# yycho0108/qpwcnet

Hardware: AMD Instinct MI355X
Metric: image-pairs/sec at 256x512 fp32 (higher is better)
Workload: dtype f32; 1 GPU; BASELINE configs[1]: full 6-level PWC-Net (qpwcnet build_flower) inference, batch 8 per GPU, 256x512 fp32, channels_last, d=4 cost volume + WarpV2; global_batch=8, batch_per_gpu=8, parallelism=dp1 (pairs sharded, RCCL all-gather of the 6 per-level EPE), hipgraph=True

## Files before the change

include/qpwc.h:

```cpp
#ifndef QPWC_H_
#define QPWC_H_

#include <stddef.h>
#include <stdint.h>

#ifdef __cplusplus
extern "C" {
#endif

#define QPWC_VERSION 200

#define QPWC_NHWC 0
#define QPWC_NCHW 1

#define QPWC_F32 0
#define QPWC_F16 1

#define QPWC_WARP_CLAMP 0
#define QPWC_WARP_TFWARP 1

#define QPWC_BCAST_B 1
#define QPWC_BCAST_H 2
#define QPWC_BCAST_W 4

// ... 138 lines not shown
int qpwc_invert_flow_fwd(const void* flow, void* out, int B, int H, int W, int layout, int dtype,
                         void* stream);

int qpwc_occlusion_fwd(const void* flow, void* out, int B, int H, int W, int layout, int dtype,
                       void* stream);

int qpwc_conv3x3_mish_fwd(const void* x, const void* weight, const void* bias, void* out, int B, int H,
                          int W, int C, int pad_h, int pad_w, void* stream);

int qpwc_conv3x3_mish_x3_fwd(const void* x, const void* weight3, const void* bias, void* out, int B, int H,
                             int W, int C, int pad_h, int pad_w, void* stream);

int qpwc_split_bf16x3_fwd(const void* src, void* out, long long n, void* stream);

int qpwc_conv3x3_mish_f16_fwd(const void* x, const void* weight, const void* bias, void* out, int B, int H,
                              int W, int C, int pad_h, int pad_w, void* stream);

int qpwc_first_conv_mish_fwd(const void* pairs, const void* weight, const void* bias, void* out, int B,
                             int H, int W, int layout, void* stream);

int qpwc_first_conv_mish_f16_fwd(const void* pairs, const void* weight, const void* bias, void* out, int B,
                                 int H, int W, int layout, void* stream);

int qpwc_conv3x3s2_mish_fwd(const void* x_padded, const void* weight, const void* bias, void* out, int B,
                            int H, int W, void* stream);

int qpwc_conv3x3s2_mish_c_fwd(const void* x_padded, const void* weight, const void* bias, void* out, int B,
                              int H, int W, int C_in, void* stream);

int qpwc_conv3x3s2_mish_x3_fwd(const void* x_padded, const void* weight3, const void* bias, void* out, int B,
                               int H, int W, int C_in, void* stream);

int qpwc_conv3x3s2_mish_f16_fwd(const void* x_padded, const void* weight, const void* bias, void* out, int B,
                                int H, int W, int C_in, void* stream);

int qpwc_upconv4x4s2_mish_fwd(const void* x, const void* weight, const void* bias, void* out, int B, int H, int W,
                              int C, int F, int64_t out_pixel_stride, void* stream);

int qpwc_upconv4x4s2_mish_x3_fwd(const void* x, const void* weight3, const void* bias, void* out, int B, int H, int W,
                                 int C, int F, int64_t out_pixel_stride, void* stream);

int qpwc_upconv4x4s2_mish_f16_fwd(const void* x, const void* weight, const void* bias, void* out, int B, int H, int W,
                                  int C, int F, int64_t out_pixel_stride, void* stream);

int qpwc_upconv4x4s2_mish_cat_fwd(const void* x, const void* weight, const void* bias, const void* skip,
                                  int64_t skip_batch_stride, int64_t skip_row_stride, int64_t skip_pixel_stride, void* out,
// ... 11 lines not shown
```

qpwcnet_amd/_hip.py:

```python
import ctypes
import os

_HERE = os.path.dirname(os.path.abspath(__file__))
LIB_PATH = os.environ.get("QPWC_HIP_LIB") or os.path.join(_HERE, "csrc", "libqpwc_hip.so")

NHWC, NCHW = 0, 1
F32, F16 = 0, 1
WARP_CLAMP, WARP_TFWARP = 0, 1
BCAST_B, BCAST_H, BCAST_W = 1, 2, 4
LOSS_FLOW_MSE_V2, LOSS_FLOW_MSE, LOSS_FLOW_FINETUNE, LOSS_AUTORESIZE_MSE = 0, 1, 2, 3

E_NULL, E_LAYOUT, E_DTYPE, E_SHAPE, E_RANGE, E_MODE, E_ALIAS, E_LAUNCH, E_ALIGN, E_STRIDE, \
    E_NODEVICE = range(-1, -12, -1)
_ARGUMENT_ERRORS = {E_NULL, E_LAYOUT, E_DTYPE, E_SHAPE, E_RANGE, E_MODE, E_ALIAS, E_ALIGN, E_STRIDE}

SYMBOLS = (
    "qpwc_version", "qpwc_last_error", "qpwc_strerror", "qpwc_build_info", "qpwc_device_copy", "qpwc_clock_probe", "qpwc_layout_transpose_fwd", "qpwc_copy_pixels_fwd",
    "qpwc_cost_volume_fwd", "qpwc_cost_volume_fwd_strided", "qpwc_warp_fwd",
    "qpwc_warp_cost_volume_fwd", "qpwc_cost_volume_kernel", "qpwc_epe_workspace_floats", "qpwc_epe_fwd",
    "qpwc_dwconv3x3_fwd", "qpwc_flow_head_param_floats", "qpwc_flow_head_fwd", "qpwc_flow_head_up_fwd", "qpwc_pointwise_bias_fwd", "qpwc_optflow_tail_fwd", "qpwc_bias_mish_fwd",
    "qpwc_upsample2x_flow_fwd", "qpwc_epe_multi_workspace_floats", "qpwc_epe_multi_fwd", "qpwc_epe_multi_mixed_fwd",
    "qpwc_cost_volume_to_flow_fwd", "qpwc_sepconv3x3_fwd", "qpwc_sepconv3x3_f16_fwd", "qpwc_bias_mish_pad_fwd", "qpwc_split_frames_pad_fwd",
    "qpwc_invert_flow_fwd", "qpwc_occlusion_fwd", "qpwc_conv3x3_mish_fwd", "qpwc_conv3x3_mish_f16_fwd", "qpwc_conv3x3_mish_x3_fwd", "qpwc_split_bf16x3_fwd", "qpwc_sepconv3x3_x3_fwd", "qpwc_conv3x3s2_mish_x3_fwd", "qpwc_upconv4x4s2_mish_x3_fwd",
    "qpwc_first_conv_mish_fwd", "qpwc_first_conv_mish_f16_fwd", "qpwc_conv3x3s2_mish_fwd", "qpwc_conv3x3s2_mish_c_fwd", "qpwc_conv3x3s2_mish_f16_fwd", "qpwc_upconv4x4s2_mish_fwd", "qpwc_upconv4x4s2_mish_f16_fwd", "qpwc_upconv4x4s2_mish_cat_fwd", "qpwc_upconv4x4s2_mish_cat_f16_fwd",
    "qpwc_cost_volume_bwd", "qpwc_warp_bwd_workspace_floats", "qpwc_warp_bwd",
    "qpwc_loss_workspace_floats", "qpwc_loss_fwd", "qpwc_loss_fwd_kernel", "qpwc_loss_bwd",
)

_lib = None


def build(verbose=False):
    import subprocess
    cmd = ["make", "-C", os.path.join(_HERE, "csrc"), "-j4"]
    if not verbose:
        cmd.append("-s")
    subprocess.check_call(cmd)
    return LIB_PATH


def lib():
    global _lib
    if _lib is not None:
        return _lib
    if not os.path.exists(LIB_PATH):
        raise RuntimeError(
            "qpwcnet_amd: {} is missing -- build it with `make -C qpwcnet_amd/csrc` or "
# ... 69 lines not shown
    L.qpwc_cost_volume_to_flow_fwd.argtypes = [vp, vp, ci, ci, ci, ci, i64, ci, ci, vp]
    L.qpwc_cost_volume_to_flow_fwd.restype = ci
    L.qpwc_sepconv3x3_f16_fwd.restype = ci
    L.qpwc_bias_mish_pad_fwd.argtypes = [vp, vp, vp, ci, ci, ci, ci, ci, ci, i64, ci, vp]
    L.qpwc_bias_mish_pad_fwd.restype = ci
    L.qpwc_split_frames_pad_fwd.argtypes = [vp, vp, ci, ci, ci, ci, ci, ci, vp]
    L.qpwc_split_frames_pad_fwd.restype = ci
    L.qpwc_invert_flow_fwd.argtypes = [vp, vp, ci, ci, ci, ci, ci, vp]
    L.qpwc_invert_flow_fwd.restype = ci
    L.qpwc_occlusion_fwd.argtypes = [vp, vp, ci, ci, ci, ci, ci, vp]
    L.qpwc_occlusion_fwd.restype = ci
    L.qpwc_conv3x3_mish_f16_fwd.argtypes = [vp, vp, vp, vp, ci, ci, ci, ci, ci, ci, vp]
    L.qpwc_conv3x3_mish_f16_fwd.restype = ci
    L.qpwc_conv3x3_mish_fwd.argtypes = [vp, vp, vp, vp, ci, ci, ci, ci, ci, ci, vp]
    L.qpwc_conv3x3_mish_fwd.restype = ci
    L.qpwc_conv3x3_mish_x3_fwd.argtypes = [vp, vp, vp, vp, ci, ci, ci, ci, ci, ci, vp]
    L.qpwc_conv3x3_mish_x3_fwd.restype = ci
    L.qpwc_split_bf16x3_fwd.argtypes = [vp, vp, i64, vp]
    L.qpwc_split_bf16x3_fwd.restype = ci
    L.qpwc_first_conv_mish_fwd.argtypes = [vp, vp, vp, vp, ci, ci, ci, ci, vp]
    L.qpwc_first_conv_mish_fwd.restype = ci
    L.qpwc_first_conv_mish_f16_fwd.argtypes = L.qpwc_first_conv_mish_fwd.argtypes
    L.qpwc_first_conv_mish_f16_fwd.restype = ci
    L.qpwc_conv3x3s2_mish_fwd.argtypes = [vp, vp, vp, vp, ci, ci, ci, vp]
    L.qpwc_conv3x3s2_mish_fwd.restype = ci
    L.qpwc_conv3x3s2_mish_c_fwd.argtypes = [vp, vp, vp, vp, ci, ci, ci, ci, vp]
    L.qpwc_conv3x3s2_mish_c_fwd.restype = ci
    L.qpwc_conv3x3s2_mish_f16_fwd.argtypes = L.qpwc_conv3x3s2_mish_c_fwd.argtypes
    L.qpwc_conv3x3s2_mish_x3_fwd.argtypes = L.qpwc_conv3x3s2_mish_c_fwd.argtypes
    L.qpwc_conv3x3s2_mish_x3_fwd.restype = ci
    L.qpwc_conv3x3s2_mish_f16_fwd.restype = ci
    L.qpwc_upconv4x4s2_mish_fwd.argtypes = [vp, vp, vp, vp, ci, ci, ci, ci, ci, i64, vp]
    L.qpwc_upconv4x4s2_mish_fwd.restype = ci
    L.qpwc_upconv4x4s2_mish_f16_fwd.argtypes = L.qpwc_upconv4x4s2_mish_fwd.argtypes
    L.qpwc_upconv4x4s2_mish_x3_fwd.argtypes = L.qpwc_upconv4x4s2_mish_fwd.argtypes
    L.qpwc_upconv4x4s2_mish_x3_fwd.restype = ci
    L.qpwc_upconv4x4s2_mish_f16_fwd.restype = ci
    L.qpwc_upconv4x4s2_mish_cat_fwd.argtypes = [vp, vp, vp, vp, i64, i64, i64, vp, ci, ci, ci, ci, ci, i64, vp]
    L.qpwc_upconv4x4s2_mish_cat_fwd.restype = ci
    L.qpwc_upconv4x4s2_mish_cat_f16_fwd.argtypes = L.qpwc_upconv4x4s2_mish_cat_fwd.argtypes
    L.qpwc_upconv4x4s2_mish_cat_f16_fwd.restype = ci
    L.qpwc_cost_volume_bwd.argtypes = [vp, vp, vp, vp, vp, vp, ci, ci, ci, ci, ci, ci, cf, vp]
    L.qpwc_cost_volume_bwd.restype = ci
    L.qpwc_warp_bwd_workspace_floats.argtypes = [ci, ci, ci, ci, ci]
    L.qpwc_warp_bwd_workspace_floats.restype = i64
    L.qpwc_warp_bwd.argtypes = [vp, vp, vp, vp, vp, vp, ci, ci, ci, ci, ci, ci, vp]
# ... 39 lines not shown
```

qpwcnet_amd/csrc/capi.hip:

```cpp
#include <stdarg.h>
#include <stdio.h>

#include "common.h"

namespace qpwc {

static thread_local char g_err[512] = "";
thread_local const char* g_dry_kernel = nullptr;
thread_local bool g_dry_run = false;

void set_error(const char* fmt, ...) {
    va_list ap;
    va_start(ap, fmt);
    vsnprintf(g_err, sizeof(g_err), fmt, ap);
    va_end(ap);
}

int check_launch(const char* what) {
    const hipError_t e = hipGetLastError();
    if (e != hipSuccess) {
        set_error("%s: %s", what, hipGetErrorString(e));
        return QPWC_E_LAUNCH;
    }
    return QPWC_OK;
// ... 52 lines not shown
int upconv4x4s2_mish_launch(const void* x, const void* weight, const void* bias, void* out, int B, int H, int W, int C,
                            int F, int out_pixel_stride, hipStream_t s, const void* skip = nullptr, int64_t skip_bs = 0,
                            int64_t skip_rs = 0, int64_t skip_ps = 0);
int upconv4x4s2_mish_f16_launch(const void* x, const void* weight, const void* bias, void* out, int B, int H, int W, int C,
                            int F, int out_pixel_stride, hipStream_t s, const void* skip = nullptr, int64_t skip_bs = 0,
                            int64_t skip_rs = 0, int64_t skip_ps = 0);
int conv3x3s2_mish_any_launch(const void* x, const void* weight, const void* bias, void* out, int B, int H, int W,
                              int CI, hipStream_t s);
int conv3x3s2_mish_f16_launch(const void* x, const void* weight, const void* bias, void* out, int B, int H, int W,
                              int CI, hipStream_t s);
int conv3x3_mish_launch(const void* x, const void* weight, const void* bias, void* out, int B, int H, int W,
                        int C, int pad_h, int pad_w, hipStream_t s);
int conv3x3_mish_x3_launch(const void* x, const void* w3, const void* bias, void* out, int B, int H, int W, int C,
                           int pad_h, int pad_w, hipStream_t s);
int split_bf16x3_launch(const void* src, void* out, int64_t n, hipStream_t s);
int conv3x3s2_mish_x3_launch(const void* x, const void* w3, const void* bias, void* out, int B, int H, int W, int CI,
                             hipStream_t s);
int upconv4x4s2_mish_x3_launch(const void* x, const void* w3, const void* bias, void* out, int B, int H, int W, int C,
                               int F, int out_pixel_stride, hipStream_t s);
int conv3x3_mish_f16_launch(const void* x, const void* weight, const void* bias, void* out, int B, int H, int W,
                        int C, int pad_h, int pad_w, hipStream_t s);
int first_conv_mish_launch(const void* x, const void* weight, const void* bias, void* out, int B, int H, int W,
                           int layout, int dtype, hipStream_t s);
int conv3x3s2_mish_launch(const void* x, const void* weight, const void* bias, void* out, int B, int H, int W,
                          hipStream_t s);
int bias_mish_launch(void* x, const void* bias, int64_t n_pixels, int C, int dtype, hipStream_t s);
int cost_volume_bwd_launch(const void* prv, const void* nxt, const void* out, const void* gout, void* gprv,
                           void* gnxt, int B, int H, int W, int C, int r, int dtype, float slope, hipStream_t s);
int warp_bwd_launch(const void* img, const void* flo, const void* gout, void* gimg, void* gflo, void* ws, int B,
                    int H, int W, int C, int dtype, int mode, hipStream_t s);
int64_t loss_workspace_floats(int n_levels);
const char* loss_fwd_kernel(int kind, int H, int W, const int* h, const int* w, int n, const void* gt);
int loss_fwd_launch(int kind, float p0, float p1, const float* gt, int B, int H, int W, int C, int layout,
                    const void* const* pred, const int* h, const int* w, const int* pred_dtype, int n, float* out,
                    void* const* dpred, void* const* gt_out, float* ws, hipStream_t s);
int loss_bwd_launch(const void* const* dpred, const float* grad_losses, void* const* grad_pred, const int64_t* n_elems,
                    const int* pred_dtype, int n, hipStream_t s);

typedef unsigned int copy_u32x4 __attribute__((ext_vector_type(4)));
__global__ __launch_bounds__(256) void device_copy_kernel(const copy_u32x4* __restrict__ src,
                                                         copy_u32x4* __restrict__ dst, int64_t n16) {
    const int64_t i = (int64_t)blockIdx.x * 256 + threadIdx.x;
    if (i < n16) __builtin_nontemporal_store(__builtin_nontemporal_load(src + i), dst + i);
}

static int fail(int code, const char* fmt, ...) {
// ... 761 lines not shown
        return fail(QPWC_E_SHAPE, "C=%d not in {16,32,64,128,256}", C);
    if (B <= 0 || H <= 0 || W <= 0 || pad_h < 0 || pad_w < 0 || pad_h > 8 || pad_w > 8)
        return fail(QPWC_E_SHAPE, "bad shape B=%d H=%d W=%d pad=%d,%d", B, H, W, pad_h, pad_w);
    if ((uintptr_t)x % 16 || (uintptr_t)weight % 16 || (uintptr_t)bias % 16 || (uintptr_t)out % 16)
        return fail(QPWC_E_ALIGN, "x, weight, bias, out must be 16-byte aligned");
    if (overlaps(out, (size_t)B * (H + pad_h) * (W + pad_w) * C * 2, x, (size_t)B * H * W * C * 2))
        return fail(QPWC_E_ALIAS, "out overlaps x");
    return conv3x3_mish_f16_launch(x, weight, bias, out, B, H, W, C, pad_h, pad_w, (hipStream_t)stream);
}

int qpwc_first_conv_mish_fwd(const void* pairs, const void* weight, const void* bias, void* out, int B,
                             int H, int W, int layout, void* stream) {
    if (!pairs || !weight || !bias || !out) return fail(QPWC_E_NULL, "null pointer argument");
    if (layout != QPWC_NHWC && layout != QPWC_NCHW) return fail(QPWC_E_LAYOUT, "Unsupported data format : %d", layout);
    if (B <= 0 || H < 2 || W < 2 || (H & 1) || (W & 1))
        return fail(QPWC_E_SHAPE, "B=%d H=%d W=%d: H and W must be even and >= 2", B, H, W);
    if ((uintptr_t)pairs % 8 || (uintptr_t)weight % 4 || (uintptr_t)bias % 16 || (uintptr_t)out % 16)
        return fail(QPWC_E_ALIGN, "pairs must be 8-byte, bias and out 16-byte aligned");
    if (overlaps(out, (size_t)2 * B * (H / 2) * (W / 2) * 16 * 4, pairs, (size_t)B * H * W * 6 * 4))
        return fail(QPWC_E_ALIAS, "out overlaps pairs");
    return first_conv_mish_launch(pairs, weight, bias, out, B, H, W, layout, QPWC_F32, (hipStream_t)stream);
}

int qpwc_first_conv_mish_f16_fwd(const void* pairs, const void* weight, const void* bias, void* out, int B,
                                 int H, int W, int layout, void* stream) {
    if (!pairs || !weight || !bias || !out) return fail(QPWC_E_NULL, "null pointer argument");
    if (layout != QPWC_NHWC && layout != QPWC_NCHW) return fail(QPWC_E_LAYOUT, "Unsupported data format : %d", layout);
    if (B <= 0 || H < 2 || W < 2 || (H & 1) || (W & 1))
        return fail(QPWC_E_SHAPE, "B=%d H=%d W=%d: H and W must be even and >= 2", B, H, W);
    if ((uintptr_t)pairs % 4 || (uintptr_t)weight % 4 || (uintptr_t)bias % 16 || (uintptr_t)out % 8)
        return fail(QPWC_E_ALIGN, "pairs must be 4-byte, bias 16-byte and out 8-byte aligned");
    if (overlaps(out, (size_t)2 * B * (H / 2) * (W / 2) * 16 * 2, pairs, (size_t)B * H * W * 6 * 2))
        return fail(QPWC_E_ALIAS, "out overlaps pairs");
    return first_conv_mish_launch(pairs, weight, bias, out, B, H, W, layout, QPWC_F16, (hipStream_t)stream);
}

int qpwc_conv3x3s2_mish_fwd(const void* x_padded, const void* weight, const void* bias, void* out, int B,
                            int H, int W, void* stream) {
    if (!x_padded || !weight || !bias || !out) return fail(QPWC_E_NULL, "null pointer argument");
    if (B <= 0 || H < 2 || W < 2 || (H & 1) || (W & 1))
        return fail(QPWC_E_SHAPE, "B=%d H=%d W=%d: H and W must be even and >= 2", B, H, W);
    if ((uintptr_t)x_padded % 16 || (uintptr_t)weight % 16 || (uintptr_t)bias % 16 || (uintptr_t)out % 16)
        return fail(QPWC_E_ALIGN, "x, weight, bias, out must be 16-byte aligned");
    if (overlaps(out, (size_t)B * (H / 2) * (W / 2) * 32 * 4, x_padded, (size_t)B * (H + 1) * (W + 1) * 16 * 4))
        return fail(QPWC_E_ALIAS, "out overlaps x");
    return conv3x3s2_mish_launch(x_padded, weight, bias, out, B, H, W, (hipStream_t)stream);
// ... 133 lines not shown
```

qpwcnet_amd/csrc/encoder.hip:

```cpp
#include "common.h"

namespace qpwc {

__device__ __forceinline__ float enc_mishf(float x) {
    const float e = __builtin_amdgcn_exp2f(fminf(x, 20.0f) * 1.4426950408889634f);
    const float t = e * (e + 2.0f);
    const float m = x * (t * __builtin_amdgcn_rcpf(t + 2.0f));
    return m;
}

typedef float f32x4e __attribute__((ext_vector_type(4)));

__device__ __forceinline__ float2 ld2(const float* p) { return *reinterpret_cast<const float2*>(p); }
__device__ __forceinline__ float2 ld2(const __half* p) { return __half22float2(*reinterpret_cast<const __half2*>(p)); }
__device__ __forceinline__ void st4q(float* p, float4 v) { *reinterpret_cast<float4*>(p) = v; }
__device__ __forceinline__ void st4q(__half* p, float4 v) {
    __half2 lo = __floats2half2_rn(v.x, v.y), hi = __floats2half2_rn(v.z, v.w);
    uint2 u;
    u.x = *reinterpret_cast<unsigned*>(&lo);
    u.y = *reinterpret_cast<unsigned*>(&hi);
    *reinterpret_cast<uint2*>(p) = u;
}

constexpr int kEcTH = 8, kEcTW = 16;
// ... 1115 lines not shown
            st4q(ob + ((int64_t)gy * Wo + gx) * 16 + 4 * g,
                 make_float4(enc_mishf(acc[r][0] + bq.x), enc_mishf(acc[r][1] + bq.y), enc_mishf(acc[r][2] + bq.z),
                             enc_mishf(acc[r][3] + bq.w)));
    }
}

int first_conv_mish_launch(const void* x, const void* weight, const void* bias, void* out, int B, int H, int W,
                           int layout, int dtype, hipStream_t s) {
    const int tiles_x = (W / 2 + kEcTW - 1) / kEcTW, tiles_y = (H / 2 + kFcTH - 1) / kFcTH;
    const int64_t nblk = (int64_t)tiles_x * tiles_y * B;
    if (nblk > INT32_MAX) {
        set_error("first_conv_mish: too many tiles");
        return QPWC_E_SHAPE;
    }
    if (dtype == QPWC_F32)
        hipLaunchKernelGGL(first_conv_mish_kernel<float>, dim3((unsigned)nblk), dim3(256), 0, s, (const float*)x,
                           (const float*)weight, (const float*)bias, (float*)out, B, H, W, tiles_x, tiles_y,
                           layout == QPWC_NCHW ? 1 : 0);
    else
        hipLaunchKernelGGL(first_conv_mish_kernel<__half>, dim3((unsigned)nblk), dim3(256), 0, s, (const __half*)x,
                           (const float*)weight, (const float*)bias, (__half*)out, B, H, W, tiles_x, tiles_y,
                           layout == QPWC_NCHW ? 1 : 0);
    return check_launch("first_conv_mish_kernel");
}

constexpr int kS2IH = 2 * kEcTH + 1;
constexpr int kS2PW = kEcTW + 1;

__global__ __launch_bounds__(256, 4) void conv3x3s2_mish_kernel(const float* __restrict__ x,
                                                                const float* __restrict__ weight,
                                                                const float* __restrict__ bias,
                                                                float* __restrict__ out, int H, int W,
                                                                int tiles_x, int tiles_y) {
    constexpr int CI = 16, CO = 32;
    __shared__ __attribute__((aligned(16))) float in_s[2 * kS2IH * kS2PW * CI];
    const int tid = threadIdx.x;
    const int wave = __builtin_amdgcn_readfirstlane(tid >> 6);
    const int lane = tid & 63, n = lane & 15, g = lane >> 4;
    const int tile = xcd_swizzle(blockIdx.x, gridDim.x);
    const int tx = tile % tiles_x, ty = (tile / tiles_x) % tiles_y, b = tile / (tiles_x * tiles_y);
    const int X0 = tx * kEcTW, Y0 = ty * kEcTH;
    const int Hp = H + 1, Wp = W + 1, Ho = H / 2, Wo = W / 2;
    const float* xb = x + (int64_t)b * Hp * Wp * CI;
    for (int idx = tid; idx < kS2IH * 33 * 4; idx += 256) {
        const int q = idx & 3, pxl = idx >> 2;
        const int row = pxl / 33, col = pxl - row * 33;
// ... 389 lines not shown
```

qpwcnet_amd/non_layers.py:

```python
import math

import torch
import torch.nn.functional as F

from . import ops
from .backend import CHANNELS_FIRST, CHANNELS_LAST, get_axis, image_data_format


def _get_axis(data_format):
    return get_axis(data_format)


def parse_image_shape(tensor, data_format=None):
    if data_format is None:
        data_format = image_data_format()
    if data_format == CHANNELS_FIRST:
        n, c, h, w = tensor.shape
    else:
        n, h, w, c = tensor.shape
    return {"n": n, "c": c, "h": h, "w": w}


def lrelu(x):
    return F.leaky_relu(x, 0.1)
# ... 202 lines not shown
            buf = torch.empty(skip.shape[:3] + (c1 + c2,), dtype=x.dtype, device=x.device)
            nb = x.shape[0] // nsplit
            for i in range(nsplit):
                yh = F.conv_transpose2d(self._nchw(x[i * nb:(i + 1) * nb]), w, None, stride=2, padding=1)
                ops.bias_mish_into(yh.permute(0, 2, 3, 1), self.p32("conv_up.bias"), buf[i * nb:(i + 1) * nb], 0)
            buf[..., c1:] = skip
            return buf
        y = F.conv_transpose2d(self._nchw(x), self.p("conv_up.weight"), None, stride=2, padding=1)
        if _hip_act_ok(y, self.data_format) and skip.shape[3] % 4 == 0:
            c1, c2 = y.shape[1], skip.shape[3]
            buf = torch.empty(skip.shape[:3] + (c1 + c2,), dtype=y.dtype, device=y.device)
            ops.bias_mish_into(y.permute(0, 2, 3, 1), self.p32("conv_up.bias"), buf, 0)
            buf[..., c1:] = skip
            return buf
        up = self._fmt(_bias_mish(y, self.p("conv_up.bias"), self.p32("conv_up.bias"), self.data_format))
        return torch.cat([up, skip], dim=self.axis)


class DownConv(_Weighted):

    def __call__(self, x):
        return self.forward_padded(x)[0]

    def forward_padded(self, x, padded_in=None, want_padded=False, after_a=None):
        if after_a is None and padded_in is not None and self._hip_s2_ok(padded_in):
            key = self.prefix + ("#taps_a" if padded_in.dtype == torch.float32 else "#taps_a_f16")
            t = self.params.get(key)
            if t is None:
                t = self.params[key] = ops.conv3x3_taps(self.p("conv_a.weight"), padded_in.dtype)
            if self.matmul == "bf16x3" and self.x3_stride2 and padded_in.dtype == torch.float32 and \
                    padded_in.shape[3] in (32, 64, 128):
                t3 = self.params.get(self.prefix + "#taps_a_x3")
                if t3 is None:
                    t3 = self.params[self.prefix + "#taps_a_x3"] = ops.split_bf16x3(t)
                after_a = ops.conv3x3s2_mish_x3(padded_in, t3, self.p32("conv_a.bias"))
            else:
                after_a = ops.conv3x3s2_mish(padded_in, t, self.p32("conv_a.bias"))
        if after_a is not None:
            y = after_a.permute(0, 3, 1, 2)
        else:
            if padded_in is not None:
                y = F.conv2d(self._nchw(padded_in), self.p("conv_a.weight"), None, stride=2)
            else:
                y = conv2d_same(self._nchw(x), self.p("conv_a.weight"), None, 2)
            y = _bias_mish(y, self.p("conv_a.bias"), self.p32("conv_a.bias"), self.data_format)
        h, w = y.shape[2], y.shape[3]
        pad_ok = want_padded and _same_pad(h, 3, 2) == (0, 1) and _same_pad(w, 3, 2) == (0, 1)
# ... 29 lines not shown
                padded_in.dtype in (torch.float32, torch.float16) and padded_in.is_contiguous() and
                padded_in.shape[3] in (16, 32, 64, 128) and
                tuple(w.shape) == (2 * padded_in.shape[3], padded_in.shape[3], 3, 3) and
                padded_in.shape[1] % 2 == 1 and padded_in.shape[2] % 2 == 1)

    def _hip_conv_ok(self, y_nchw):
        return (self.hip_conv and y_nchw.dtype in (torch.float32, torch.float16) and
                y_nchw.shape[1] in (16, 32, 64, 128, 256) and _hip_act_ok(y_nchw, self.data_format))

    def first_layer(self, pairs, pairs_format=None):
        w = self.p("conv_a.weight")
        pf = self.data_format if pairs_format is None else pairs_format
        hh, ww, cc = (pairs.shape[2], pairs.shape[3], pairs.shape[1]) if pf == CHANNELS_FIRST else \
            (pairs.shape[1], pairs.shape[2], pairs.shape[3])
        if not (self.hip_conv and self.data_format == CHANNELS_LAST and pairs.is_cuda and
                pairs.dtype in (torch.float32, torch.float16) and tuple(w.shape) == (16, 3, 3, 3) and
                hh % 2 == 0 and ww % 2 == 0 and cc == 6):
            return None
        key = self.prefix + "#taps_a"
        t = self.params.get(key)
        if t is None:
            t = self.params[key] = ops.first_conv_taps(w)
        return ops.first_conv_mish(pairs.contiguous(), t, self.p32("conv_a.bias"), pf)

    def _taps(self, dtype=torch.float32):
        key = self.prefix + ("#taps" if dtype == torch.float32 else "#taps_f16")
        t = self.params.get(key)
        if t is None:
            t = self.params[key] = (ops.conv3x3_taps(self.p("conv_aa.weight"), dtype),
                                    ops.conv3x3_taps(self.p("conv_b.weight"), dtype))
        return t

    def _taps_x3(self):
        key = self.prefix + "#taps_x3"
        t = self.params.get(key)
        if t is None:
            t = self.params[key] = tuple(ops.split_bf16x3(w) for w in self._taps(torch.float32))
        return t


class OptFlow(_Weighted):

    BN_EPS = 1e-3
    matmul = "f32"
    x3_filters = (128, 64)
    x3_min_pixels = 8 * 64 * 128
# ... 353 lines not shown
```

qpwcnet_amd/ops.py:

```python
import ctypes

import torch

from . import _hip
from .backend import CHANNELS_FIRST, CHANNELS_LAST, get_axis

_DTYPES = {torch.float32: _hip.F32, torch.float16: _hip.F16}


class KernelTimer:

    def __init__(self):
        self.records = []

    def __enter__(self):
        global _TIMER
        self._prev, _TIMER = _TIMER, self
        return self

    def __exit__(self, *exc):
        global _TIMER
        _TIMER = self._prev
        return False

# ... 922 lines not shown

def first_conv_mish(pairs, taps, bias, data_format=CHANNELS_LAST):
    _check_tensor("pairs", pairs)
    cf = data_format == CHANNELS_FIRST
    get_axis(data_format)
    if pairs.shape[1 if cf else 3] != 6 or pairs.dtype not in (torch.float32, torch.float16) or not pairs.is_contiguous():
        raise ValueError("pairs must be a dense fp32 / fp16 (B,H,W,6) / (B,6,H,W) tensor")
    if cf:
        B, _, H, W = pairs.shape
    else:
        B, H, W, _ = pairs.shape
    if tuple(taps.shape) != (9, 16, 4) or taps.dtype != torch.float32 or not taps.is_contiguous() or \
            bias.numel() != 16 or bias.dtype != torch.float32:
        raise ValueError("taps must be fp32 (9,16,4), bias fp32 (16)")
    out = torch.empty((2 * B, H // 2, W // 2, 16), dtype=pairs.dtype, device=pairs.device)
    fn = _hip.lib().qpwc_first_conv_mish_fwd if pairs.dtype == torch.float32 else _hip.lib().qpwc_first_conv_mish_f16_fwd
    with torch.cuda.device(out.device), _timed("first_conv_mish", (B, H, W, 6)):
        rc = fn(pairs.data_ptr(), taps.data_ptr(), bias.data_ptr(), out.data_ptr(), B, H, W,
                _hip.NCHW if cf else _hip.NHWC, _stream(out))
    _hip.check(rc)
    return out


def conv3x3s2_mish(x_padded, taps, bias):
    _check_tensor("x", x_padded)
    ci = x_padded.shape[3]
    if x_padded.dtype not in (torch.float32, torch.float16) or not x_padded.is_contiguous() or ci not in (16, 32, 64, 128):
        raise ValueError("conv3x3s2_mish needs a dense fp32 / fp16 (B,H+1,W+1,C) tensor, C in {16,32,64,128}")
    B, Hp, Wp, _ = x_padded.shape
    H, W = Hp - 1, Wp - 1
    if tuple(taps.shape) != (9, 2 * ci, ci) or taps.dtype != x_padded.dtype or not taps.is_contiguous() or \
            bias.numel() != 2 * ci or bias.dtype != torch.float32:
        raise ValueError("taps must be (9,{},{}) of the input's dtype, bias fp32 ({})".format(2 * ci, ci, 2 * ci))
    out = torch.empty((B, H // 2, W // 2, 2 * ci), dtype=x_padded.dtype, device=x_padded.device)
    f16 = x_padded.dtype == torch.float16
    fn = _hip.lib().qpwc_conv3x3s2_mish_f16_fwd if f16 else _hip.lib().qpwc_conv3x3s2_mish_c_fwd
    with torch.cuda.device(out.device), _timed("conv3x3s2_mish_f16" if f16 else "conv3x3s2_mish", (B, H, W, ci)):
        rc = fn(x_padded.data_ptr(), taps.data_ptr(), bias.data_ptr(), out.data_ptr(), B, H, W, ci, _stream(out))
    _hip.check(rc)
    return out


def conv3x3s2_mish_x3(x_padded, taps3, bias):
    _check_tensor("x", x_padded)
    ci = x_padded.shape[3]
    if x_padded.dtype != torch.float32 or not x_padded.is_contiguous() or ci not in (32, 64, 128):
# ... 124 lines not shown
```

qpwcnet_amd/pwcnet.py:

```python
import numpy as np
import torch

from . import ops
from .backend import CHANNELS_FIRST, CHANNELS_LAST, get_axis, image_data_format
from .non_layers import (DownConv, Downsample, Flow, Flower, FrameInterpolate, Split, UpConv, UpFlow,
                         Upsample)
from .synth import DEC_FILTERS, ENC_FILTERS, make_interpolator_weights, make_weights


def encoder(layers, img_prv, img_nxt, output_features=False):
    f = img_prv
    feats_prv = [f]
    for l in layers:
        f = l(f)
        feats_prv.append(f)
    f = img_nxt
    feats_nxt = [f]
    for l in layers:
        f = l(f)
        feats_nxt.append(f)
    if output_features:
        return feats_prv, feats_nxt
    return feats_prv[-1], feats_nxt[-1]

# ... 48 lines not shown
class QpwcNet:

    def __init__(self, weights, train=True, input_shape=(256, 512), data_format=None,
                 use_tfa=True, device="cuda", dtype=torch.float32, fused=None, hip_optflow=True,
                 batch_frames=True, overlap_streams=True, internal_channels_last=True):
        self.data_format = image_data_format() if data_format is None else data_format
        self.axis = get_axis(self.data_format)
        self.train = train
        self.batch_frames = bool(batch_frames)
        self.overlap_streams = bool(overlap_streams)
        self._side = None
        self._sides = []
        self.dec_stream_of = (0, 0, 0, 0)
        self.prefill_skips = False
        self.skip_copy_first = ()
        self._prefilled = {}
        self.dec_chunks = (2, 4, 4, 1)
        self.dec_chunk_max_frames = 64
        self.dec_chunk_max_pixels = 64 * 256 * 512
        self.capture_order = ("F0", "D0", "D1", "D2", "D3", "F1", "F2", "F3", "F4")
        self.dec_after_flow = {}
        self._matmul = "f32"
        self.skip_redundant_join = True
        self.input_shape = tuple(input_shape)
        self.device = torch.device(device)
        self.dtype = dtype
        self._df = CHANNELS_LAST if (self.data_format == CHANNELS_FIRST and self.batch_frames and hip_optflow and
                                     internal_channels_last and self.device.type == "cuda") else self.data_format
        self.params = {}
        for k, v in weights.items():
            t = torch.as_tensor(np.asarray(v)).to(self.device, dtype)
            if t.dim() == 4 and self._df == CHANNELS_LAST:
                t = t.contiguous(memory_format=torch.channels_last)
            self.params[k] = t
        df = self._df
        self.split = Split(2, axis=self.axis, data_format=df)
        self.enc = [DownConv(self.params, "enc.{}.".format(i), data_format=df)
                    for i in range(len(ENC_FILTERS))]
        self.dec = [UpConv(self.params, "dec.{}.".format(i), data_format=df)
                    for i in range(len(DEC_FILTERS))]
        self.flow = Flow(self.params, "flow.", use_tfa=use_tfa, hip_optflow=hip_optflow, data_format=df)
        self.upflows = [UpFlow(self.params, "upflow.{}.".format(i), use_tfa=use_tfa, fused=fused,
                               hip_optflow=hip_optflow, data_format=df)
                        for i in range(len(DEC_FILTERS))]
        if self._df != self.data_format:
            for blk in [self.flow] + self.upflows:
# ... 56 lines not shown

    def _prefill(self, li, f):
        i = len(self.dec) - 1 - li
        if i < 0 or self.dec_stream_of[i] != 0:
            return
        main = torch.cuda.current_stream()
        if self._side is None:
            self._side = torch.cuda.Stream(device=f.device)
        if not self._sides:
            self._sides.append(self._side)
        side = self._sides[0]
        c_in = ENC_FILTERS[-1] if i == 0 else DEC_FILTERS[i - 1] + ENC_FILTERS[-1 - i]
        ev = torch.cuda.Event()
        ev.record(main)
        side.wait_event(ev)
        with torch.cuda.stream(side):
            buf = self.dec[i].prefill_skip(f, c_in)
        if buf is not None:
            f.record_stream(side)
            self._prefilled[i] = buf

    def _encode_stacked(self, inputs, prefill=False):
        h, w = self.input_shape
        first = self.enc[0].first_layer(inputs, self.data_format)
        split_axis = self.axis
        if first is None and self._df != self.data_format:
            inputs = ops.layout_transpose(inputs, self._df)
            split_axis = get_axis(self._df)
        if first is not None:
            f, padded = inputs, None
        elif (self._df == CHANNELS_LAST and inputs.is_cuda and h % 2 == 0 and w % 2 == 0 and
                inputs.dtype in (torch.float32, torch.float16)):
            padded = ops.split_frames_pad(inputs, 1, 1)
            f = padded[:, :h, :w, :]
        else:
            f, padded = torch.cat(torch.chunk(inputs, 2, dim=split_axis), dim=0), None
        encs = [f]
        for li, l in enumerate(self.enc):
            f, padded = l.forward_padded(f, padded, want_padded=li + 1 < len(self.enc),
                                         after_a=first if li == 0 else None)
            encs.append(f)
            if prefill and li + 1 < len(self.enc):
                self._prefill(li, f)
        return encs

    def _forward_stacked(self, encs, nb, overlap):
        if overlap:
            return self._forward_two_streams(encs, nb)
        f, decs, i = encs[-1], [], -2
        for l in self.dec:
            f = l.cat_skip(f, encs[i])
            i -= 1
            decs.append(f)
        flo = self.flow((encs[-1][:nb], encs[-1][nb:]))
        flos = [flo]
        for i, upflow in enumerate(self.upflows):
            flo = upflow((decs[i][:nb], decs[i][nb:], self._up(flo)))
            flos.append(flo)
        flos.append(self._up(flo, last=True))
        return flos if self.train else flos[-1]

    def _forward_two_streams(self, encs, nb):
        main = torch.cuda.current_stream()
# ... 186 lines not shown
```

Before: 7314 pairs/s.

## Fuse first encoder conv_a and conv_aa into one MFMA kernel with LDS halo

Adds a HIP kernel that computes the first stride-2 conv (conv_a) on a haloed tile and keeps its Mish output in shared memory. The kernel then applies the 3x3 conv_aa plus Mish on MFMA and writes only the second layer's output. This removes one full-resolution intermediate write and read plus a kernel launch at the largest encoder level. In exchange the kernel recomputes halo pixels of the first layer, uses more shared memory and registers, and only covers fp32 channels_last inputs with the expected weight shapes.

```diff
diff --git a/include/qpwc.h b/include/qpwc.h
--- a/include/qpwc.h
+++ b/include/qpwc.h
@@ -184,6 +184,10 @@
 int qpwc_first_conv_mish_f16_fwd(const void* pairs, const void* weight, const void* bias, void* out, int B,
                                  int H, int W, int layout, void* stream);
 
+int qpwc_first_conv3x3_mish_fwd(const void* pairs, const void* weight_a, const void* bias_a, const void* weight_aa,
+                                const void* bias_aa, void* out, int B, int H, int W, int pad_h, int pad_w,
+                                void* stream);
+
 int qpwc_conv3x3s2_mish_fwd(const void* x_padded, const void* weight, const void* bias, void* out, int B,
                             int H, int W, void* stream);
 
diff --git a/qpwcnet_amd/_hip.py b/qpwcnet_amd/_hip.py
--- a/qpwcnet_amd/_hip.py
+++ b/qpwcnet_amd/_hip.py
@@ -22,7 +22,7 @@
     "qpwc_upsample2x_flow_fwd", "qpwc_epe_multi_workspace_floats", "qpwc_epe_multi_fwd", "qpwc_epe_multi_mixed_fwd",
     "qpwc_cost_volume_to_flow_fwd", "qpwc_sepconv3x3_fwd", "qpwc_sepconv3x3_f16_fwd", "qpwc_bias_mish_pad_fwd", "qpwc_split_frames_pad_fwd",
     "qpwc_invert_flow_fwd", "qpwc_occlusion_fwd", "qpwc_conv3x3_mish_fwd", "qpwc_conv3x3_mish_f16_fwd", "qpwc_conv3x3_mish_x3_fwd", "qpwc_split_bf16x3_fwd", "qpwc_sepconv3x3_x3_fwd", "qpwc_conv3x3s2_mish_x3_fwd", "qpwc_upconv4x4s2_mish_x3_fwd",
-    "qpwc_first_conv_mish_fwd", "qpwc_first_conv_mish_f16_fwd", "qpwc_conv3x3s2_mish_fwd", "qpwc_conv3x3s2_mish_c_fwd", "qpwc_conv3x3s2_mish_f16_fwd", "qpwc_upconv4x4s2_mish_fwd", "qpwc_upconv4x4s2_mish_f16_fwd", "qpwc_upconv4x4s2_mish_cat_fwd", "qpwc_upconv4x4s2_mish_cat_f16_fwd",
+    "qpwc_first_conv_mish_fwd", "qpwc_first_conv_mish_f16_fwd", "qpwc_first_conv3x3_mish_fwd", "qpwc_conv3x3s2_mish_fwd", "qpwc_conv3x3s2_mish_c_fwd", "qpwc_conv3x3s2_mish_f16_fwd", "qpwc_upconv4x4s2_mish_fwd", "qpwc_upconv4x4s2_mish_f16_fwd", "qpwc_upconv4x4s2_mish_cat_fwd", "qpwc_upconv4x4s2_mish_cat_f16_fwd",
     "qpwc_cost_volume_bwd", "qpwc_warp_bwd_workspace_floats", "qpwc_warp_bwd",
     "qpwc_loss_workspace_floats", "qpwc_loss_fwd", "qpwc_loss_fwd_kernel", "qpwc_loss_bwd",
 )
@@ -138,6 +138,8 @@
     L.qpwc_first_conv_mish_fwd.restype = ci
     L.qpwc_first_conv_mish_f16_fwd.argtypes = L.qpwc_first_conv_mish_fwd.argtypes
     L.qpwc_first_conv_mish_f16_fwd.restype = ci
+    L.qpwc_first_conv3x3_mish_fwd.argtypes = [vp, vp, vp, vp, vp, vp, ci, ci, ci, ci, ci, vp]
+    L.qpwc_first_conv3x3_mish_fwd.restype = ci
     L.qpwc_conv3x3s2_mish_fwd.argtypes = [vp, vp, vp, vp, ci, ci, ci, vp]
     L.qpwc_conv3x3s2_mish_fwd.restype = ci
     L.qpwc_conv3x3s2_mish_c_fwd.argtypes = [vp, vp, vp, vp, ci, ci, ci, ci, vp]
diff --git a/qpwcnet_amd/csrc/capi.hip b/qpwcnet_amd/csrc/capi.hip
--- a/qpwcnet_amd/csrc/capi.hip
+++ b/qpwcnet_amd/csrc/capi.hip
@@ -98,6 +98,8 @@
                         int C, int pad_h, int pad_w, hipStream_t s);
 int first_conv_mish_launch(const void* x, const void* weight, const void* bias, void* out, int B, int H, int W,
                            int layout, int dtype, hipStream_t s);
+int first_conv3x3_mish_launch(const void* x, const void* w1, const void* b1, const void* w2, const void* b2, void* out,
+                              int B, int H, int W, int pad_h, int pad_w, hipStream_t s);
 int conv3x3s2_mish_launch(const void* x, const void* weight, const void* bias, void* out, int B, int H, int W,
                           hipStream_t s);
 int bias_mish_launch(void* x, const void* bias, int64_t n_pixels, int C, int dtype, hipStream_t s);
@@ -905,6 +907,22 @@
     return first_conv_mish_launch(pairs, weight, bias, out, B, H, W, layout, QPWC_F32, (hipStream_t)stream);
 }
 
+int qpwc_first_conv3x3_mish_fwd(const void* pairs, const void* weight_a, const void* bias_a, const void* weight_aa,
+                                const void* bias_aa, void* out, int B, int H, int W, int pad_h, int pad_w,
+                                void* stream) {
+    if (!pairs || !weight_a || !bias_a || !weight_aa || !bias_aa || !out)
+        return fail(QPWC_E_NULL, "null pointer argument");
+    if (B <= 0 || H < 2 || W < 2 || (H & 1) || (W & 1) || pad_h < 0 || pad_w < 0 || pad_h > 8 || pad_w > 8)
+        return fail(QPWC_E_SHAPE, "B=%d H=%d W=%d pad=%d,%d: H and W must be even and >= 2", B, H, W, pad_h, pad_w);
+    if ((uintptr_t)pairs % 16 || (uintptr_t)weight_a % 16 || (uintptr_t)bias_a % 16 || (uintptr_t)weight_aa % 16 ||
+        (uintptr_t)bias_aa % 16 || (uintptr_t)out % 16)
+        return fail(QPWC_E_ALIGN, "pairs, weights, biases and out must be 16-byte aligned");
+    if (overlaps(out, (size_t)2 * B * (H / 2 + pad_h) * (W / 2 + pad_w) * 16 * 4, pairs, (size_t)B * H * W * 6 * 4))
+        return fail(QPWC_E_ALIAS, "out overlaps pairs");
+    return first_conv3x3_mish_launch(pairs, weight_a, bias_a, weight_aa, bias_aa, out, B, H, W, pad_h, pad_w,
+                                     (hipStream_t)stream);
+}
+
 int qpwc_first_conv_mish_f16_fwd(const void* pairs, const void* weight, const void* bias, void* out, int B,
                                  int H, int W, int layout, void* stream) {
     if (!pairs || !weight || !bias || !out) return fail(QPWC_E_NULL, "null pointer argument");
diff --git a/qpwcnet_amd/csrc/encoder.hip b/qpwcnet_amd/csrc/encoder.hip
--- a/qpwcnet_amd/csrc/encoder.hip
+++ b/qpwcnet_amd/csrc/encoder.hip
@@ -1161,6 +1161,183 @@
                            (const float*)weight, (const float*)bias, (__half*)out, B, H, W, tiles_x, tiles_y,
                            layout == QPWC_NCHW ? 1 : 0);
     return check_launch("first_conv_mish_kernel");
+}
+
+constexpr int kFfIH = 2 * (kEcTH + 2) + 1, kFfIW = 2 * kEcHW + 1;
+constexpr int kFfRowQ = (kFfIW * 6 + 3) / 4, kFfRow = 256;
+constexpr int kFfNP = (kFfIH + 3) / 4, kFfPatch = kFfNP * 4 * kFfRow;
+static_assert(kFfRowQ <= 56 && 4 * 56 + 2 * 6 + 1 <= kFfRow, "k-slot 3 reads zeros at floats 224 .. 236 of a row");
+typedef unsigned u32x4f __attribute__((ext_vector_type(4)));
+constexpr int kFfNG = (kEcNH + 15) / 16;
+constexpr int kFfGW = kFfNG / 2;
+static_assert(kFfNG % 2 == 0, "two waves share a frame's halo groups");
+constexpr int kFfPix = 24, kFfHalo = 2 * kEcNH * kFfPix;
+__device__ __forceinline__ int ff_halo(int f, int hp, int g) { return (f * kEcNH + hp) * kFfPix + 4 * g; }
+
+__global__ __launch_bounds__(256, 4) void first_conv3x3_mish_kernel(const float* __restrict__ x,
+                                                                    const float* __restrict__ w1,
+                                                                    const float* __restrict__ b1,
+                                                                    const float* __restrict__ w2,
+                                                                    const float* __restrict__ b2,
+                                                                    float* __restrict__ out, int B, int H, int W,
+                                                                    int pad_h, int pad_w, int tiles_x, int tiles_y) {
+    __shared__ __attribute__((aligned(16))) float smem_s[kFfPatch > kFfHalo ? kFfPatch : kFfHalo];
+    float* const patch_s = smem_s;
+    float* const halo_s = smem_s;
+    const int tid = threadIdx.x;
+    const int wave = __builtin_amdgcn_readfirstlane(tid >> 6);
+    const int lane = tid & 63, n = lane & 15, g = lane >> 4;
+    const int tile = xcd_swizzle(blockIdx.x, gridDim.x);
+    const int tx = tile % tiles_x, ty = (tile / tiles_x) % tiles_y, b = tile / (tiles_x * tiles_y);
+    const int X0 = tx * kEcTW, Y0 = ty * kEcTH;
+    const int Hl = H / 2, Wl = W / 2;
+    const int Ho = Hl + pad_h, Wo = Wl + pad_w;
+    const __amdgpu_buffer_rsrc_t rx = __builtin_amdgcn_make_buffer_rsrc(
+        const_cast<float*>(x) + (int64_t)b * H * W * 6, 0, H * W * 24, 0x00020000);
+    const int e0 = 12 * X0 - 12 + 4 * lane;
+    const unsigned coff = (lane < kFfRowQ && (unsigned)e0 < (unsigned)(6 * W)) ? 4u * (unsigned)e0 : kEwOob;
+    constexpr int NP = kFfNP;
+    u32x4f pv[NP];
+#pragma unroll
+    for (int it = 0; it < NP; ++it) {
+        const int row = wave + 4 * it, gy = 2 * Y0 - 2 + row;
+        const bool rin = row < kFfIH && (unsigned)gy < (unsigned)H;
+        pv[it] = __builtin_amdgcn_raw_buffer_load_b128(rx, rin ? coff : kEwOob, rin ? gy * W * 24 : 0, 0);
+    }
+    __builtin_amdgcn_sched_barrier(0);
+    float wv[9];
+#pragma unroll
+    for (int k = 0; k < 9; ++k) wv[k] = w1[(k * 16 + n) * 4 + g];
+    const float4 bq1 = *reinterpret_cast<const float4*>(b1 + 4 * g);
+    __builtin_amdgcn_sched_barrier(0);
+#pragma unroll
+    for (int it = 0; it < NP; ++it) *reinterpret_cast<u32x4f*>(patch_s + 4 * (tid + 256 * it)) = pv[it];
+    __syncthreads();
+
+    f32x4e wld[9];
+    float4 bq2;
+    {
+        const int f = wave >> 1;
+        int hpv[kFfGW], pb[kFfGW];
+        const int gstep = g < 3 ? 12 : 0, goff = g < 3 ? 3 * f + g : 4 * 56;
+        bool inside[kFfGW];
+#pragma unroll
+        for (int j = 0; j < kFfGW; ++j) {
+            hpv[j] = 16 * (kFfGW * (wave & 1) + j) + n;
+            const int hp = hpv[j] < kEcNH ? hpv[j] : kEcNH - 1;
+            const int hy = hp / kEcHW, hx = hp - hy * kEcHW;
+            const int ly = Y0 - 1 + hy, lx = X0 - 1 + hx;
+            inside[j] = ly >= 0 && ly < Hl && lx >= 0 && lx < Wl;
+            pb[j] = 2 * hy * kFfRow + hx * gstep + goff;
+        }
+        f32x4e acc[kFfGW];
+#pragma unroll
+        for (int j = 0; j < kFfGW; ++j) acc[j] = f32x4e{0.f, 0.f, 0.f, 0.f};
+        float vb[2][kFfGW];
+        auto read_tap = [&](float (&v)[kFfGW], int k) __attribute__((always_inline)) {
+            const int ky = k / 3, kx = k - 3 * ky;
+#pragma unroll
+            for (int j = 0; j < kFfGW; ++j) v[j] = patch_s[pb[j] + ky * kFfRow + kx * 6];
+        };
+        read_tap(vb[0], 0);
+#pragma unroll
+        for (int k = 0; k < 9; ++k) {
+            if (k + 1 < 9) read_tap(vb[(k + 1) & 1], k + 1);
+            __builtin_amdgcn_sched_barrier(0);
+#pragma unroll
+            for (int j = 0; j < kFfGW; ++j)
+                acc[j] = __builtin_amdgcn_mfma_f32_16x16x4f32(wv[k], vb[k & 1][j], acc[j], 0, 0, 0);
+#pragma unroll
+            for (int j = 0; j < kFfGW; ++j) ew_pin_agpr(acc[j]);
+            __builtin_amdgcn_sched_barrier(0);
+        }
+#pragma unroll
+        for (int k = 0; k < 9; ++k) wld[k] = *reinterpret_cast<const f32x4e*>(w2 + ((int64_t)k * 16 + n) * 16 + 4 * g);
+        bq2 = *reinterpret_cast<const float4*>(b2 + 4 * g);
+        float4 hv[kFfGW];
+#pragma unroll
+        for (int j = 0; j < kFfGW; ++j) {
+            hv[j] = make_float4(enc_mishf(acc[j][0] + bq1.x), enc_mishf(acc[j][1] + bq1.y),
+                                enc_mishf(acc[j][2] + bq1.z), enc_mishf(acc[j][3] + bq1.w));
+            if (!inside[j]) hv[j] = make_float4(0.f, 0.f, 0.f, 0.f);
+        }
+        __syncthreads();
+#pragma unroll
+        for (int j = 0; j < kFfGW; ++j)
+            if (hpv[j] < kEcNH)
+                *reinterpret_cast<float4*>(halo_s + ff_halo(f, hpv[j], g)) = hv[j];
+    }
+    __syncthreads();
+
+    f32x4e acc[4];
+#pragma unroll
+    for (int a = 0; a < 4; ++a) acc[a] = f32x4e{0.f, 0.f, 0.f, 0.f};
+    const float* hb = halo_s + ff_halo(0, 2 * wave * kEcHW + n, g);
+    f32x4e bv[2][4];
+    auto read_tap = [&](f32x4e (&v)[4], int k) __attribute__((always_inline)) {
+        const int ky = k / 3, kx = k - 3 * ky;
+#pragma unroll
+        for (int a = 0; a < 4; ++a) {
+            const int dhp = ((a & 1) + ky) * kEcHW + kx;
+            v[a] = *reinterpret_cast<const f32x4e*>(hb + ff_halo(a >> 1, dhp, 0));
+        }
+    };
+    read_tap(bv[0], 0);
+#pragma unroll
+    for (int k = 0; k < 9; ++k) {
+        if (k + 1 < 9) read_tap(bv[(k + 1) & 1], k + 1);
+        __builtin_amdgcn_sched_barrier(0);
+#pragma unroll
+        for (int tt = 0; tt < 4; ++tt)
+#pragma unroll
+            for (int a = 0; a < 4; ++a)
+                acc[a] = __builtin_amdgcn_mfma_f32_16x16x4f32(wld[k][tt], bv[k & 1][a][tt], acc[a], 0, 0, 0);
+#pragma unroll
+        for (int a = 0; a < 4; ++a) ew_pin_agpr(acc[a]);
+        __builtin_amdgcn_sched_barrier(0);
+    }
+#pragma unroll
+    for (int a = 0; a < 4; ++a) {
+        const int gy = Y0 + 2 * wave + (a & 1), gx = X0 + n;
+        float* ob = out + (int64_t)((a >> 1) * B + b) * Ho * Wo * 16;
+        if (gy < Hl && gx < Wl)
+            *reinterpret_cast<float4*>(ob + ((int64_t)gy * Wo + gx) * 16 + 4 * g) =
+                make_float4(enc_mishf(acc[a][0] + bq2.x), enc_mishf(acc[a][1] + bq2.y),
+                            enc_mishf(acc[a][2] + bq2.z), enc_mishf(acc[a][3] + bq2.w));
+    }
+    if ((pad_w > 0 && X0 + kEcTW >= Wl) || (pad_h > 0 && Y0 + kEcTH >= Hl)) {
+        for (int f = 0; f < 2; ++f) {
+            float* ob = out + (int64_t)(f * B + b) * Ho * Wo * 16;
+            if (pad_w > 0 && X0 + kEcTW >= Wl) {
+                for (int i = tid; i < kEcTH * pad_w * 4; i += 256) {
+                    const int q = i % 4, r = i / 4, col = r % pad_w, row = r / pad_w;
+                    const int gy = Y0 + row;
+                    if (gy < Hl) *reinterpret_cast<float4*>(ob + ((int64_t)gy * Wo + Wl + col) * 16 + 4 * q) = make_float4(0.f, 0.f, 0.f, 0.f);
+                }
+            }
+            if (pad_h > 0 && Y0 + kEcTH >= Hl) {
+                const int x_end = (X0 + kEcTW >= Wl) ? Wo : X0 + kEcTW;
+                for (int i = tid; i < pad_h * (x_end - X0) * 4; i += 256) {
+                    const int q = i % 4, r = i / 4, col = r % (x_end - X0), row = r / (x_end - X0);
+                    *reinterpret_cast<float4*>(ob + ((int64_t)(Hl + row) * Wo + X0 + col) * 16 + 4 * q) = make_float4(0.f, 0.f, 0.f, 0.f);
+                }
+            }
+        }
+    }
+}
+
+int first_conv3x3_mish_launch(const void* x, const void* w1, const void* b1, const void* w2, const void* b2, void* out,
+                              int B, int H, int W, int pad_h, int pad_w, hipStream_t s) {
+    const int tiles_x = (W / 2 + kEcTW - 1) / kEcTW, tiles_y = (H / 2 + kEcTH - 1) / kEcTH;
+    const int64_t nblk = (int64_t)tiles_x * tiles_y * B;
+    if (nblk > INT32_MAX || (int64_t)H * W * 24 > INT32_MAX) {
+        set_error("first_conv3x3_mish: too many tiles or a pair of 2 GiB or more");
+        return QPWC_E_SHAPE;
+    }
+    hipLaunchKernelGGL(first_conv3x3_mish_kernel, dim3((unsigned)nblk), dim3(256), 0, s, (const float*)x,
+                       (const float*)w1, (const float*)b1, (const float*)w2, (const float*)b2, (float*)out, B, H, W,
+                       pad_h, pad_w, tiles_x, tiles_y);
+    return check_launch("first_conv3x3_mish_kernel");
 }
 
 constexpr int kS2IH = 2 * kEcTH + 1;
diff --git a/qpwcnet_amd/non_layers.py b/qpwcnet_amd/non_layers.py
--- a/qpwcnet_amd/non_layers.py
+++ b/qpwcnet_amd/non_layers.py
@@ -248,7 +248,13 @@
     def __call__(self, x):
         return self.forward_padded(x)[0]
 
-    def forward_padded(self, x, padded_in=None, want_padded=False, after_a=None):
+    def forward_padded(self, x, padded_in=None, want_padded=False, after_a=None, after_aa=None):
+        if after_aa is not None:
+            h, w = after_aa.shape[1], after_aa.shape[2]
+            pad_ok = want_padded and _same_pad(h, 3, 2) == (0, 1) and _same_pad(w, 3, 2) == (0, 1)
+            pad = 1 if pad_ok else 0
+            y2 = ops.conv3x3_mish(after_aa, self._taps(after_aa.dtype)[1], self.p32("conv_b.bias"), pad, pad)
+            return (y2[:, :h, :w, :], y2) if pad_ok else (y2, None)
         if after_a is None and padded_in is not None and self._hip_s2_ok(padded_in):
             key = self.prefix + ("#taps_a" if padded_in.dtype == torch.float32 else "#taps_a_f16")
             t = self.params.get(key)
@@ -324,6 +330,21 @@
         if t is None:
             t = self.params[key] = ops.first_conv_taps(w)
         return ops.first_conv_mish(pairs.contiguous(), t, self.p32("conv_a.bias"), pf)
+
+    def first_two_layers(self, pairs, pairs_format=None):
+        w = self.p("conv_a.weight")
+        pf = self.data_format if pairs_format is None else pairs_format
+        if not (self.hip_conv and self.matmul == "f32" and self.data_format == CHANNELS_LAST and pf == CHANNELS_LAST and
+                pairs.is_cuda and pairs.dtype == torch.float32 and tuple(w.shape) == (16, 3, 3, 3) and
+                tuple(self.p("conv_aa.weight").shape) == (16, 16, 3, 3) and
+                pairs.shape[1] % 2 == 0 and pairs.shape[2] % 2 == 0 and pairs.shape[3] == 6):
+            return None
+        key = self.prefix + "#taps_a"
+        t = self.params.get(key)
+        if t is None:
+            t = self.params[key] = ops.first_conv_taps(w)
+        return ops.first_conv3x3_mish(pairs.contiguous(), t, self.p32("conv_a.bias"), self._taps()[0],
+                                      self.p32("conv_aa.bias"))
 
     def _taps(self, dtype=torch.float32):
         key = self.prefix + ("#taps" if dtype == torch.float32 else "#taps_f16")
diff --git a/qpwcnet_amd/ops.py b/qpwcnet_amd/ops.py
--- a/qpwcnet_amd/ops.py
+++ b/qpwcnet_amd/ops.py
@@ -968,6 +968,26 @@
     return out
 
 
+def first_conv3x3_mish(pairs, taps_a, bias_a, taps_aa, bias_aa, pad_h=0, pad_w=0):
+    _check_tensor("pairs", pairs)
+    if pairs.dim() != 4 or pairs.shape[3] != 6 or pairs.dtype != torch.float32 or not pairs.is_contiguous():
+        raise ValueError("pairs must be a dense fp32 (B,H,W,6) tensor")
+    B, H, W, _ = pairs.shape
+    for name, t, shape in (("taps_a", taps_a, (9, 16, 4)), ("taps_aa", taps_aa, (9, 16, 16))):
+        if tuple(t.shape) != shape or t.dtype != torch.float32 or not t.is_cuda or not t.is_contiguous():
+            raise ValueError("{} must be a dense fp32 {} device tensor".format(name, shape))
+    for name, t in (("bias_a", bias_a), ("bias_aa", bias_aa)):
+        if t.numel() != 16 or t.dtype != torch.float32 or not t.is_cuda:
+            raise ValueError("{} must be an fp32 (16) device tensor".format(name))
+    out = torch.empty((2 * B, H // 2 + pad_h, W // 2 + pad_w, 16), dtype=torch.float32, device=pairs.device)
+    with torch.cuda.device(out.device), _timed("first_conv3x3_mish", (B, H, W, 6)):
+        rc = _hip.lib().qpwc_first_conv3x3_mish_fwd(pairs.data_ptr(), taps_a.data_ptr(), bias_a.data_ptr(),
+                                                     taps_aa.data_ptr(), bias_aa.data_ptr(), out.data_ptr(), B, H, W,
+                                                     int(pad_h), int(pad_w), _stream(out))
+    _hip.check(rc)
+    return out
+
+
 def conv3x3s2_mish(x_padded, taps, bias):
     _check_tensor("x", x_padded)
     ci = x_padded.shape[3]
diff --git a/qpwcnet_amd/pwcnet.py b/qpwcnet_amd/pwcnet.py
--- a/qpwcnet_amd/pwcnet.py
+++ b/qpwcnet_amd/pwcnet.py
@@ -94,6 +94,7 @@
         self.dec_after_flow = {}
         self._matmul = "f32"
         self.skip_redundant_join = True
+        self.fuse_first_layer = True
         self.input_shape = tuple(input_shape)
         self.device = torch.device(device)
         self.dtype = dtype
@@ -196,7 +197,8 @@
 
     def _encode_stacked(self, inputs, prefill=False):
         h, w = self.input_shape
-        first = self.enc[0].first_layer(inputs, self.data_format)
+        first2 = self.enc[0].first_two_layers(inputs, self.data_format) if self.fuse_first_layer else None
+        first = first2 if first2 is not None else self.enc[0].first_layer(inputs, self.data_format)
         split_axis = self.axis
         if first is None and self._df != self.data_format:
             inputs = ops.layout_transpose(inputs, self._df)
@@ -212,7 +214,8 @@
         encs = [f]
         for li, l in enumerate(self.enc):
             f, padded = l.forward_padded(f, padded, want_padded=li + 1 < len(self.enc),
-                                         after_a=first if li == 0 else None)
+                                         after_a=first if li == 0 and first2 is None else None,
+                                         after_aa=first2 if li == 0 else None)
             encs.append(f)
             if prefill and li + 1 < len(self.enc):
                 self._prefill(li, f)
```

Result: no change. 7368 pairs/s, median of 6 (+0.7%).
